# haiciyang/LaDiffCodec

Hardware: AMD Instinct MI355X
Metric: audio-sec decoded / wall-sec, 16kHz 3kbps 50-step DDPM (higher is better)
Workload: dtype bf16; 1 GPU; LaDiffCodec 3 kbps, diff_dims=256, enc_ratios 8 4, 50-step DDPM, batch=32x2.4 s utterances per GPU; global_batch=32, latent_len=1200, denoise_steps=50, rccl_ranks=1, batches_in_flight=1, parallelism=dp1 (utterance-sharded, no data-path collective)

## Files before the change

ladiffcodec_amd/csrc/attention.hip:

```cpp
#include <algorithm>

#include "ldc_kernels.h"
#include "ldc_math.h"

namespace ldc {

__device__ __forceinline__ float abf2f(unsigned short h) { return __uint_as_float(((unsigned)h) << 16); }
__device__ __forceinline__ unsigned short af2bf(float f) { return hw_bf16(f); }
template <typename T>
__device__ __forceinline__ float ld1(const void* p, size_t i);
template <>
__device__ __forceinline__ float ld1<float>(const void* p, size_t i) { return reinterpret_cast<const float*>(p)[i]; }
template <>
__device__ __forceinline__ float ld1<__bf16>(const void* p, size_t i) {
  return abf2f(reinterpret_cast<const unsigned short*>(p)[i]);
}
template <typename T>
__device__ __forceinline__ void st1(void* p, size_t i, float v);
template <>
__device__ __forceinline__ void st1<float>(void* p, size_t i, float v) { reinterpret_cast<float*>(p)[i] = v; }
template <>
__device__ __forceinline__ void st1<__bf16>(void* p, size_t i, float v) {
  reinterpret_cast<unsigned short*>(p)[i] = af2bf(v);
}
// ... 274 lines not shown
    acc = mfma_bf16(af[0], bq[0], acc);
    acc = mfma_bf16(af[1], bq[1], acc);
    if (n < L) {
      unsigned short* orow = out + ((size_t)b * L + n) * HD + h * D;
#pragma unroll
      for (int rr = 0; rr < 4; ++rr) {
        const unsigned lo = (unsigned)af2bf(acc[4 * rr]) | ((unsigned)af2bf(acc[4 * rr + 1]) << 16);
        const unsigned hi = (unsigned)af2bf(acc[4 * rr + 2]) | ((unsigned)af2bf(acc[4 * rr + 3]) << 16);
        *reinterpret_cast<uint2*>(orow + 8 * rr + 4 * g) = n < Lv ? make_uint2(lo, hi) : make_uint2(0u, 0u);
      }
    }
  }
}


__device__ __forceinline__ float reduce16_over32(const float (&v)[16], int lane) {
  float a8[8], a4[4], a2[2];
  const bool b4 = lane & 16, b3 = lane & 8, b2 = lane & 4, b1 = lane & 2;
#pragma unroll
  for (int k = 0; k < 8; ++k) a8[k] = (b4 ? v[8 + k] : v[k]) + __shfl_xor(b4 ? v[k] : v[8 + k], 16);
#pragma unroll
  for (int k = 0; k < 4; ++k) a4[k] = (b3 ? a8[4 + k] : a8[k]) + __shfl_xor(b3 ? a8[k] : a8[4 + k], 8);
#pragma unroll
  for (int k = 0; k < 2; ++k) a2[k] = (b2 ? a4[2 + k] : a4[k]) + __shfl_xor(b2 ? a4[k] : a4[2 + k], 4);
  float a1 = (b1 ? a2[1] : a2[0]) + __shfl_xor(b1 ? a2[0] : a2[1], 2);
  a1 += __shfl_xor(a1, 1);
  return a1;
}

template <int C>
__global__ __launch_bounds__(256) void linattn_tail_mfma_kernel(const unsigned short* qkv, const float* ws, size_t ws_stride, float scale,
                                                                const unsigned short* wo, int n_pad, const float* bias, const float* gain,
                                                                const unsigned short* resid, unsigned short* out, int L, unsigned* fail_flag) {
  constexpr int D = 32, HD = 128, R = 32, CPW = C / 4, NT = CPW / 32;
  constexpr int AP = HD + 8;
  constexpr int TP = CPW * 4 + 16;
  extern __shared__ __attribute__((aligned(16))) char smem[];
  unsigned short* sA = reinterpret_cast<unsigned short*>(smem);
  float* sred = reinterpret_cast<float*>(smem + (size_t)R * AP * 2);
  float* srow = sred + 4 * R;
  char* strans = smem + (size_t)R * AP * 2 + (size_t)5 * R * 4;
  const int b = blockIdx.y, tid = threadIdx.x;
  const int w = tid >> 6, lane = tid & 63, i32 = lane & 31, g = lane >> 5;
  const int r0 = blockIdx.x * R;
  const float* wsb = ws + (size_t)b * ws_stride;
  const int colw = w * CPW + i32;
  uint4 bfr[8][NT];
#pragma unroll
  for (int ks = 0; ks < 8; ++ks)
#pragma unroll
    for (int j = 0; j < NT; ++j)
      bfr[ks][j] = *reinterpret_cast<const uint4*>(wo + ((size_t)(ks >> 1) * n_pad + colw + 32 * j) * 32 + (ks & 1) * 16 + 8 * g);
  float bv[NT], gv[NT];
#pragma unroll
  for (int j = 0; j < NT; ++j) { bv[j] = bias[colw + 32 * j]; gv[j] = gain[colw + 32 * j]; }
  {
    const int h = w;
    const int n = r0 + i32;
    uint4 qq[2];
#pragma unroll
    for (int sx = 0; sx < 2; ++sx) {
      if (n < L) qq[sx] = *reinterpret_cast<const uint4*>(qkv + ((size_t)b * L + n) * (3 * HD) + h * D + 16 * sx + 8 * g);
      else qq[sx] = make_uint4(0, 0, 0, 0);
    }
    uint4 af[2];
    bool ks_bad = false;
#pragma unroll
    for (int sx = 0; sx < 2; ++sx) {
      unsigned wv[4];
#pragma unroll
      for (int m = 0; m < 8; m += 2) {
        const int d0 = 16 * sx + 8 * g + m;
        const float ks0 = wsb[HD + h * D + d0], ks1 = wsb[HD + h * D + d0 + 1];
        ks_bad |= !(ks0 >= kLinattnKsumMin && ks0 < kLinattnKsumMax) | !(ks1 >= kLinattnKsumMin && ks1 < kLinattnKsumMax);
        const float c0 = wsb[2 * HD + (size_t)h * D * D + d0 * D + i32] * (scale / ks0);
        const float c1 = wsb[2 * HD + (size_t)h * D * D + (d0 + 1) * D + i32] * (scale / ks1);
        wv[m >> 1] = (unsigned)af2bf(c0) | ((unsigned)af2bf(c1) << 16);
      }
      af[sx] = make_uint4(wv[0], wv[1], wv[2], wv[3]);
    }
    if (ks_bad && fail_flag) __hip_atomic_store(fail_flag, kDevFailCtxRange, __ATOMIC_RELAXED, __HIP_MEMORY_SCOPE_SYSTEM);
    float x[16];
    float mx = -INFINITY;
#pragma unroll
    for (int sx = 0; sx < 2; ++sx) {
      const unsigned wv[4] = {qq[sx].x, qq[sx].y, qq[sx].z, qq[sx].w};
#pragma unroll
      for (int m = 0; m < 4; ++m) {
        x[8 * sx + 2 * m] = abf2f((unsigned short)(wv[m] & 0xffffu));
        x[8 * sx + 2 * m + 1] = abf2f((unsigned short)(wv[m] >> 16));
      }
    }
#pragma unroll
    for (int m = 0; m < 16; ++m) mx = fmaxf(mx, x[m]);
    mx = fmaxf(mx, __shfl_xor(mx, 32));
    float sum = 0.f;
#pragma unroll
    for (int m = 0; m < 16; ++m) { x[m] = __expf(x[m] - mx); sum += x[m]; }
    sum += __shfl_xor(sum, 32);
    const float inv = 1.0f / sum;
    uint4 bq[2];
#pragma unroll
    for (int sx = 0; sx < 2; ++sx) {
      unsigned wv[4];
#pragma unroll
      for (int m = 0; m < 4; ++m)
        wv[m] = (unsigned)af2bf(x[8 * sx + 2 * m] * inv) | ((unsigned)af2bf(x[8 * sx + 2 * m + 1] * inv) << 16);
      bq[sx] = make_uint4(wv[0], wv[1], wv[2], wv[3]);
    }
    lf32x16 acc1;
#pragma unroll
    for (int r = 0; r < 16; ++r) acc1[r] = 0.f;
    acc1 = mfma_bf16(af[0], bq[0], acc1);
    acc1 = mfma_bf16(af[1], bq[1], acc1);
    unsigned short* arow = sA + (size_t)i32 * AP + h * D;
#pragma unroll
    for (int rr = 0; rr < 4; ++rr) {
      const unsigned lo = (unsigned)af2bf(acc1[4 * rr]) | ((unsigned)af2bf(acc1[4 * rr + 1]) << 16);
      const unsigned hi = (unsigned)af2bf(acc1[4 * rr + 2]) | ((unsigned)af2bf(acc1[4 * rr + 3]) << 16);
      *reinterpret_cast<uint2*>(arow + 8 * rr + 4 * g) = make_uint2(lo, hi);
    }
  }
  __syncthreads();
  lf32x16 acc[NT];
#pragma unroll
  for (int j = 0; j < NT; ++j)
#pragma unroll
    for (int r = 0; r < 16; ++r) acc[j][r] = 0.f;
#pragma unroll
  for (int ks = 0; ks < 8; ++ks) {
    const uint4 afr = *reinterpret_cast<const uint4*>(sA + (size_t)i32 * AP + 16 * ks + 8 * g);
#pragma unroll
    for (int j = 0; j < NT; ++j) acc[j] = mfma_bf16(afr, bfr[ks][j], acc[j]);
  }
  constexpr int LPR = CPW / 4;
  constexpr int RPS = 64 / LPR;
  constexpr int NSW = R / RPS;
  const int rsub = lane / LPR, piece = lane % LPR;
  uint2 rres[NSW];
#pragma unroll
  for (int sw = 0; sw < NSW; ++sw) {
    const int n = r0 + sw * RPS + rsub;
    rres[sw] = n < L ? *reinterpret_cast<const uint2*>(resid + ((size_t)b * L + n) * C + w * CPW + piece * 4) : make_uint2(0, 0);
  }
#pragma unroll
  for (int j = 0; j < NT; ++j)
#pragma unroll
    for (int r = 0; r < 16; ++r) acc[j][r] += bv[j];
  const int rr = i32 >> 1;
  const int my_row = (rr & 3) + 8 * (rr >> 2) + 4 * g;
  {
    float v[16];
#pragma unroll
    for (int r = 0; r < 16; ++r) {
      float sacc = 0.f;
#pragma unroll
      for (int j = 0; j < NT; ++j) sacc += acc[j][r];
      v[r] = sacc;
    }
    const float tot = reduce16_over32(v, lane);
    if ((lane & 1) == 0) sred[w * R + my_row] = tot;
  }
  __syncthreads();
  if (tid < R) srow[tid] = (sred[tid] + sred[R + tid] + sred[2 * R + tid] + sred[3 * R + tid]) * (1.0f / (float)C);
  __syncthreads();
  float mean[16];
#pragma unroll
  for (int r = 0; r < 16; ++r) mean[r] = srow[(r & 3) + 8 * (r >> 2) + 4 * g];
  {
    float v[16];
#pragma unroll
    for (int r = 0; r < 16; ++r) {
      float sacc = 0.f;
#pragma unroll
      for (int j = 0; j < NT; ++j) { const float d = acc[j][r] - mean[r]; sacc = fmaf(d, d, sacc); }
      v[r] = sacc;
    }
    const float tot = reduce16_over32(v, lane);
    if ((lane & 1) == 0) sred[w * R + my_row] = tot;
  }
  __syncthreads();
  if (tid < R) srow[tid] = rsqrtf((sred[tid] + sred[R + tid] + sred[2 * R + tid] + sred[3 * R + tid]) * (1.0f / (float)C) + 1e-5f);
  __syncthreads();
  char* tw = strans + (size_t)w * R * TP;
#pragma unroll
  for (int r = 0; r < 16; ++r) {
    const int row = (r & 3) + 8 * (r >> 2) + 4 * g;
    const float rstd = srow[row];
#pragma unroll
    for (int j = 0; j < NT; ++j)
      reinterpret_cast<float*>(tw + (size_t)row * TP)[32 * j + i32] = (acc[j][r] - mean[r]) * rstd * gv[j];
  }
#pragma unroll
  for (int sw = 0; sw < NSW; ++sw) {
    const int row = sw * RPS + rsub;
    const int n = r0 + row;
    const float4 y = *reinterpret_cast<const float4*>(tw + (size_t)row * TP + piece * 16);
    const float o0 = y.x + abf2f((unsigned short)(rres[sw].x & 0xffffu)), o1 = y.y + abf2f((unsigned short)(rres[sw].x >> 16));
    const float o2 = y.z + abf2f((unsigned short)(rres[sw].y & 0xffffu)), o3 = y.w + abf2f((unsigned short)(rres[sw].y >> 16));
    const uint2 o = make_uint2((unsigned)af2bf(o0) | ((unsigned)af2bf(o1) << 16), (unsigned)af2bf(o2) | ((unsigned)af2bf(o3) << 16));
    if (n < L) *reinterpret_cast<uint2*>(out + ((size_t)b * L + n) * C + w * CPW + piece * 4) = o;
  }
}

template <int C>
static hipError_t launch_tail_cfg(const void* qkv, const float* ws, size_t wss, float scale, const void* wo, int n_pad, const float* bias,
                                  const float* gain, const void* resid, void* out, int B, int L, unsigned* fail_flag, hipStream_t s) {
  constexpr int R = 32, CPW = C / 4;
  const size_t lds = (size_t)R * (128 + 8) * 2 + (size_t)5 * R * 4 + (size_t)4 * R * (CPW * 4 + 16);
  auto kern = linattn_tail_mfma_kernel<C>;
  static bool lds_opt_in = false;
  if (!lds_opt_in) {
    hipError_t e = hipFuncSetAttribute(reinterpret_cast<const void*>(kern), hipFuncAttributeMaxDynamicSharedMemorySize, 160 * 1024);
    if (e != hipSuccess) return e;
    lds_opt_in = true;
  }
  hipLaunchKernelGGL(kern, dim3((L + R - 1) / R, B), dim3(256), lds, s, reinterpret_cast<const unsigned short*>(qkv), ws, wss, scale,
                     reinterpret_cast<const unsigned short*>(wo), n_pad, bias, gain, reinterpret_cast<const unsigned short*>(resid),
                     reinterpret_cast<unsigned short*>(out), L, fail_flag);
  return hipGetLastError();
}

bool linattn_tail_supported(int dt, int heads, int dim_head, int C) {
  return dt == DT_BF16 && heads == 4 && dim_head == 32 && (C == 256 || C == 512 || C == 1024);
}

hipError_t launch_linattn_ctx(int dt, const void* qkv, float* ws, int B, int L, int heads, int dim_head, hipStream_t s) {
  if (dt != DT_BF16 || heads != 4 || dim_head != 32) return hipErrorInvalidValue;
  const size_t wss = linattn_ws_per_item(heads, dim_head);
  hipLaunchKernelGGL(linattn_ctx_mfma_kernel<64>, dim3((L + 63) / 64, B), dim3(256), 0, s, reinterpret_cast<const unsigned short*>(qkv), ws, L, wss,
                     static_cast<const int*>(nullptr), 0);
  return hipGetLastError();
}

hipError_t launch_linattn_tail(int dt, const void* qkv, const float* ws, const void* wo_packed, int n_pad, const float* bias, const float* gain,
                               const void* resid, void* out, int B, int L, int heads, int dim_head, int C, unsigned* fail_flag, hipStream_t s) {
  if (!linattn_tail_supported(dt, heads, dim_head, C) || !bias || !gain || !resid) return hipErrorInvalidValue;
  const size_t wss = linattn_ws_per_item(heads, dim_head);
  const float scale = 1.0f / sqrtf((float)dim_head);
  if (C == 256) return launch_tail_cfg<256>(qkv, ws, wss, scale, wo_packed, n_pad, bias, gain, resid, out, B, L, fail_flag, s);
  if (C == 512) return launch_tail_cfg<512>(qkv, ws, wss, scale, wo_packed, n_pad, bias, gain, resid, out, B, L, fail_flag, s);
  return launch_tail_cfg<1024>(qkv, ws, wss, scale, wo_packed, n_pad, bias, gain, resid, out, B, L, fail_flag, s);
}

size_t linattn_ws_floats_per_item(int heads, int dim_head) { return linattn_ws_per_item(heads, dim_head); }

hipError_t launch_linattn_kmax(int dt, const void* qkv, float* ws, int B, int L, int heads, int dim_head, hipStream_t s, const int* lens, int shift) {
  const int HD = heads * dim_head;
  if (dim_head != 32 || HD > 256 || 256 % HD) return hipErrorInvalidValue;
  const size_t wss = linattn_ws_per_item(heads, dim_head);
  hipError_t e = hipMemsetAsync(ws, 0, (size_t)B * wss * sizeof(float), s);
  if (e != hipSuccess) return e;
  const int rpb = 128;
  if (dt == DT_F32) hipLaunchKernelGGL(linattn_kmax_kernel<float>, dim3((L + rpb - 1) / rpb, B), dim3(256), 0, s, qkv, ws, L, HD, rpb, wss, lens, shift);
  else hipLaunchKernelGGL(linattn_kmax_kernel<__bf16>, dim3((L + rpb - 1) / rpb, B), dim3(256), 0, s, qkv, ws, L, HD, rpb, wss, lens, shift);
  return hipGetLastError();
}
// ... 130 lines not shown
```

ladiffcodec_amd/csrc/ldc_api.cpp:

```cpp
#include "ldc_internal.h"

long long g_device_syncs = 0;

static thread_local char g_err[1024] = "";
int fail(int code, const char* fmt, ...) {
  va_list ap;
  va_start(ap, fmt);
  vsnprintf(g_err, sizeof(g_err), fmt, ap);
  va_end(ap);
  return code;
}

extern "C" const char* ldc_last_error(void) { return g_err; }
extern "C" const char* ldc_version(void) { return "ladiffcodec-amd 0.1 (gfx950)"; }



static std::vector<float> fold_weight_norm(const HostTensor& g, const HostTensor& v) {
  const size_t n0 = (size_t)v.shape[0], inner = v.numel() / n0;
  std::vector<float> w(v.numel());
  for (size_t i = 0; i < n0; ++i) {
    double s = 0;
    for (size_t j = 0; j < inner; ++j) s += (double)v.data[i * inner + j] * v.data[i * inner + j];
    const float nrm = (float)sqrt(s);
// ... 780 lines not shown
  LDC_OPT("ends_join", c->ends_join, false, 0, 1)
  LDC_OPT("split_init", c->split_init, true, 0, 1)
  LDC_OPT("side_streams", c->side_streams, true, 0, 1)
  LDC_OPT("serial_parts", c->serial_parts, false, 0, 1)
  LDC_OPT("stream_calib", c->calib, false, 0, 1)
  LDC_OPT("merge_advance", c->merge_advance, true, 0, 1)
  LDC_OPT("fuse_gn_stats", c->fuse_gn_stats, true, 0, 1)
  LDC_OPT("fuse_gn_epi", c->fuse_gn_epi, true, 0, 1)
  LDC_OPT("gn_epi_min_l", c->gn_epi_min_l, true, 0, 1 << 30)
  LDC_OPT("gn_epi_max_tiles", c->gn_epi_max_tiles, true, 0, 1 << 30)
  LDC_OPT("fold_res", c->fold_res, true, 0, 1)
  LDC_OPT("fold_ln", c->fold_ln, true, 0, 1)
  LDC_OPT("fuse_kmax", c->fuse_kmax, true, 0, 1)
  LDC_OPT("fuse_ln", c->fuse_ln, true, 0, 1)
  LDC_OPT("fuse_attn_tail", c->fuse_attn_tail, true, 0, 1)
  LDC_OPT("fold_ctx", c->fold_ctx, true, 0, 1)
  LDC_OPT("conv_lean", c->tune.lean, true, 0, 1)
  LDC_OPT("lean_all", c->tune.lean_all, true, 0, 1)
  LDC_OPT("ring3_tiles", c->tune.ring3_tiles, true, 0, 1 << 30)
  LDC_OPT("ring3_wgs", c->tune.ring3_wgs, true, 1, 3)
  LDC_OPT("ring3_window", c->tune.ring3_window, true, 0, 1)
  LDC_OPT("ring3_window_tiles", c->tune.ring3_window_tiles, true, 0, 1 << 30)
  LDC_OPT("conv_generic", c->tune.force_generic, true, 0, 1)
  LDC_OPT("conv_small_tiles", c->tune.small_max, true, 0, 1 << 30)
  LDC_OPT("conv_splitk", c->tune.splitk, true, 0, 4)
  LDC_OPT("sk_tiles", c->tune.sk_tiles, true, 0, 1 << 30)
  LDC_OPT("sk_u2", c->tune.sk_u2, true, 0, 1 << 30)
  LDC_OPT("sk_u3", c->tune.sk_u3, true, 0, 1 << 30)
  LDC_OPT("conv_mfast", c->tune.m_fastest, true, 0, 2)
  LDC_OPT("conv_debug", c->tune.debug, true, 0, 255)
// ... 1543 lines not shown
```

ladiffcodec_amd/csrc/ldc_api_tuning.cpp:

```cpp
#include "ldc_internal.h"

static int round_up(int v, int m) { return (v + m - 1) / m * m; }

extern "C" int ldc_sconv1d(ldc_ctx* c, const float* x, int B, int Cin, int L, const float* w_host, const float* b_host,
                           int Cout, int k, int stride, int dilation, int causal, int pre_elu, float* y, void* stream) {
  if (!c || !x || !w_host || !y) return fail(LDC_E_INVALID, "null argument");
  if (B <= 0 || Cin <= 0 || L <= 0 || Cout <= 0 || k <= 0 || stride <= 0 || dilation <= 0) return fail(LDC_E_INVALID, "bad sizes");
  HIPCHK(hipSetDevice(c->device));
  hipStream_t s = pick_stream(c, stream);
  const int cp = round_up(Cin, 16);
  std::vector<float> wp((size_t)Cout * cp * k, 0.f);
  for (int o = 0; o < Cout; ++o)
    for (int i = 0; i < Cin; ++i)
      for (int t = 0; t < k; ++t) wp[((size_t)o * cp + i) * k + t] = w_host[((size_t)o * Cin + i) * k + t];
  DevMem keep;
  std::swap(keep.ptrs, c->wmem.ptrs);
  ConvLayer ly;
  ConvSpec sp;
  sp.dt = DT_F32; sp.cin1 = cp; sp.cout = Cout; sp.k = k; sp.stride = stride; sp.dil = dilation;
  const int padding_total = (k - 1) * dilation - (stride - 1);
  sp.pad_left = causal ? padding_total : padding_total - padding_total / 2;
  sp.pad_mode = PAD_REFLECT; sp.pre_act = pre_elu ? ACT_ELU : ACT_NONE;
  int rc = make_conv(c, sp, wp.data(), b_host, &ly);
  std::swap(keep.ptrs, c->wmem.ptrs);
// ... 698 lines not shown
    std::swap(keep.ptrs, c->wmem.ptrs);
    c->w8 = saved_w8;
    LDCCHK(rc);
    LDCCHK(keep.alloc(&r_cl, (size_t)B * L * C * es));
    HIPCHK(launch_to_cl(dt, resid, r_cl, B, C, L, nullptr, 0, 0.f, s));
  }
  HIPCHK(launch_to_cl(dt, qkv, q_cl, B, 3 * HD, L, nullptr, 0, 0.f, s));
  if (kind == 0) {
    HIPCHK(launch_linattn(dt, q_cl, o_cl, (float*)ws, B, L, H, D, false, s));
  } else if (kind == 1) {
    HIPCHK(launch_linattn_kmax(dt, q_cl, (float*)ws, B, L, H, D, s));
    HIPCHK(launch_linattn(dt, q_cl, o_cl, (float*)ws, B, L, H, D, true, s));
  } else if (kind == 2) {
    HIPCHK(launch_linattn_kmax(dt, q_cl, (float*)ws, B, L, H, D, s));
    HIPCHK(launch_linattn_ctx(dt, q_cl, (float*)ws, B, L, H, D, s));
    HIPCHK(launch_linattn_tail(dt, q_cl, (const float*)ws, to_out.w, to_out.n_pad, to_out.bias, d_gain, r_cl, o_cl, B, L, H, D, C, c->dev_flag_dev, s));
  } else {
    HIPCHK(launch_attn_full(dt, q_cl, o_cl, B, L, H, D, s));
  }
  HIPCHK(launch_from_cl(dt, o_cl, out, B, Co, L, nullptr, 0, 0.f, s));
  HIPCHK(hipStreamSynchronize(s));
  return check_dev_flag(c);
}

extern "C" int ldc_conv_compare_fp8(ldc_ctx* c, int B, int L, int cin1, int cin2, int cout, int k, int stride, int ups, int with_gn,
                                    int with_colmax, double* max_abs_diff, double* max_abs_ref, double* max_rel_stat) {
  if (!c || !max_abs_diff || !max_abs_ref || !max_rel_stat) return fail(LDC_E_INVALID, "bad arguments");
  if ((cin1 % 64) || (cin2 % 64)) return fail(LDC_E_INVALID, "fp8 inputs need channel counts that are multiples of 64");
  HIPCHK(hipSetDevice(c->device));
  const int cin = cin1 + cin2;
  std::vector<float> w((size_t)cout * cin * k), bias(cout);
// ... 242 lines not shown
```

ladiffcodec_amd/csrc/ldc_internal.h:

```cpp
#pragma once
#include "../../include/ladiffcodec.h"

#include <hip/hip_runtime.h>
#include <math.h>
#include <stdarg.h>
#include <stdio.h>
#include <string.h>

#include <algorithm>
#include <chrono>
#include <functional>
#include <map>
#include <memory>
#include <set>
#include <string>
#include <vector>

#include "ldc_kernels.h"
#include "ldc_windows.h"
#include "plan_passes.h"
static_assert(kGnSumFloats == ldc::kGnPad, "plan_passes.h sizes the GroupNorm sums by the kernels' padding");

extern long long g_device_syncs;
inline hipError_t counted_device_sync() {
// ... 240 lines not shown
  int fp8_act = 1;
  int part_graphs = 1;
  double host_graph_ms = 0, host_wait_ms = 0;
  long long host_graph_launches = 0;
  hipStream_t side_stream[kMaxParts] = {nullptr, nullptr, nullptr, nullptr};
  hipEvent_t ev_side_fork[kMaxParts] = {nullptr, nullptr, nullptr, nullptr}, ev_side_join[kMaxParts] = {nullptr, nullptr, nullptr, nullptr};
  int side_streams = 0;
  int fuse_kmax = 1;
  int fuse_ln = 1;
  int coop_launch = 0;
  int lstm_xcd = 1;
  int num_cus = 256;
  int xcd_resident[2] = {0, 0};
  int coop_resident[2] = {0, 0};
  int fuse_attn_tail = 1;
  int fold_ctx = 1;
  static constexpr int kFlowRing = 32;
  hipEvent_t flow_ev[kFlowRing] = {};
  unsigned long long flow_n = 0;
  int flow_depth = 8;
  int fuse_gn_stats = 1;
  int gn_epi_max_tiles = 1300;
  int gn_epi_min_l = 0;
  int fold_ln = 1;
  int fold_res = 1;
  int fuse_gn_epi = 1;
  ConvTune tune;
  int lstm_stream_only = 0;
  int serial_parts = 0;
  int graph_steps = 0;
// ... 191 lines not shown
```

ladiffcodec_amd/csrc/ldc_kernels.h:

```cpp
#pragma once
#include <hip/hip_runtime.h>
#include <stdint.h>

#include "ldc_windows.h"

namespace ldc {

enum { DT_F32 = 0, DT_BF16 = 1, DT_FP8 = 2 };
enum { ACT_NONE = 0, ACT_SILU = 1, ACT_ELU = 2, ACT_TANH = 3, ACT_GELU = 4, ACT_SIGMOID = 5, ACT_RELU = 6 };
enum { PAD_ZERO = 0, PAD_REFLECT = 1 };
static constexpr int kGnPad = 16;

inline size_t dt_size(int dt) { return dt == DT_F32 ? 4 : (dt == DT_FP8 ? 1 : 2); }

struct ConvLayer {
  int dt = DT_F32;
  int cin1 = 0, cin2 = 0;
  int n = 0;
  int n_pad = 0;
  int bn = 128;
  int taps = 1, stride = 1, dil = 1, pad_left = 0, ups = 0, pad_mode = PAD_ZERO;
  int pre_act = ACT_NONE, post_act = ACT_NONE;
  int tr_stride = 0, tr_cout = 0, tr_trim_left = 0;
  void* w = nullptr;
// ... 88 lines not shown
                           int ss_stride, const int* t_ptr, int act, hipStream_t s, void* y_ln = nullptr, const float* ln_g = nullptr, int out8 = 0,
                           const int* lens = nullptr, int shift = 0,
                           int t_stride = 0, int t_rows = 0);
bool gn_apply_ln_fusable(int C);
hipError_t launch_ln_rows(int dt, const void* x, void* y, const void* residual, const float* g, int rows, int C,
                          hipStream_t s, int out8 = 0, const int* lens = nullptr, int shift = 0, int L = 0);
hipError_t launch_mask_rows(int dt, void* x, int B, int L, int C, const int* lens, int shift, hipStream_t s);
hipError_t launch_act(int dt, const void* x, void* y, int64_t n, int act, hipStream_t s, int out8 = 0);

hipError_t launch_linattn(int dt, const void* qkv, void* out, float* ctx_ws, int B, int L, int heads, int dim_head,
                          bool kmax_fused, hipStream_t s, const int* lens = nullptr, int shift = 0, bool ws_zeroed = false);
size_t linattn_ws_floats_per_item(int heads, int dim_head);
bool linattn_tail_supported(int dt, int heads, int dim_head, int C);
hipError_t launch_linattn_ctx(int dt, const void* qkv, float* ctx_ws, int B, int L, int heads, int dim_head, hipStream_t s);
hipError_t launch_linattn_tail(int dt, const void* qkv, const float* ctx_ws, const void* wo_packed, int n_pad, const float* bias, const float* gain,
                               const void* resid, void* out, int B, int L, int heads, int dim_head, int C, unsigned* fail_flag, hipStream_t s);
hipError_t launch_linattn_kmax(int dt, const void* qkv, float* ctx_ws, int B, int L, int heads, int dim_head, hipStream_t s,
                               const int* lens = nullptr, int shift = 0);
constexpr float kLinattnKClamp = 60.0f;
constexpr float kLinattnKsumMin = 7.888609052210118e-31f;
constexpr float kLinattnKsumMax = 1.0e26f;
constexpr unsigned kDevFailCtxRange = 4u;
hipError_t launch_attn_full(int dt, const void* qkv, void* out, int B, int L, int heads, int dim_head, hipStream_t s, const int* lens = nullptr,
                            int shift = 0);

hipError_t launch_to_cl(int dt, const float* x_bcl, void* y_blc, int B, int C, int L, const float* maxabs,
                        int maxabs_per_item, float eps, hipStream_t s);
hipError_t launch_from_cl(int dt, const void* x_blc, float* y_bcl, int B, int C, int L, const float* maxabs,
                          int maxabs_per_item, float eps, hipStream_t s);
hipError_t launch_maxabs(int dt, const void* x, int B, int64_t n_per_item, int per_item, float* maxabs,
                         hipStream_t s);
// ... 192 lines not shown
```

ladiffcodec_amd/csrc/unet_plan.cpp:

```cpp
#include "ldc_internal.h"

bool gn_apply_fp8_ok(int C) { return C % 8 == 0 && C / 8 <= 256 && 256 % (C / 8) == 0 && C <= 2048; }

void* PlanBuilder::act(int rows, int C) {
  pl->act_bytes += (double)rows * C * es;
  return ar->alloc((size_t)rows * C * es);
}
const int* PlanBuilder::lens() const { return pl->ragged ? (pl->lens ? pl->lens : reinterpret_cast<const int*>(16)) : nullptr; }
int PlanBuilder::level(int L) const {
  int sh = 0;
  while ((L << sh) < pl->L) ++sh;
  return sh;
}
void PlanBuilder::mask(void* y, int L, int C) {
  if (!pl->ragged) return;
  const int dt = c->dt, Bn = B, sh = level(L);
  const int* ln = pl->lens;
  info = "mask_rows_c" + std::to_string(C) + "_L" + std::to_string(L);
  add([=](hipStream_t s) { return launch_mask_rows(dt, y, Bn, L, C, ln, sh, s); }, false, 0, LDC_CLASS_ELEMENTWISE, 0);
}
void PlanBuilder::mark(int kind) {
  pl->step.push_back({[](hipStream_t) { return hipSuccess; }, kind, LDC_CLASS_OTHER, 0, 0, "-"});
}
void PlanBuilder::add(std::function<hipError_t(hipStream_t)> f, bool is_conv, double flops, int cls, double bytes) {
// ... 212 lines not shown
        2.0 * rows * a.dim * es);
  if (linear) {
    const size_t wss = linattn_ws_floats_per_item(H, Dh);
    if (!ln && c->fuse_kmax && c->fuse_attn_tail && !a.out.w8 && linattn_tail_supported(dt, H, Dh, a.dim)) {
      ln_rowstat_next = rowstat;
      if (lnf && c->fold_ctx && c->tune.lean && !c->tune.force_generic && dt == DT_BF16 && a.qkv_ctx.w && hid == 128 && a.dim % 64 == 0) {
        qkv_ctx_next = ws; qkv_ctx_stride_next = (int)wss;
        conv(a.qkv_ctx, xn, nullptr, qkv, nullptr, L, L);
      } else {
        conv(qkv_ly, xn, nullptr, qkv, nullptr, L, L, nullptr, reinterpret_cast<unsigned*>(ws), hid, 2 * hid, (int)wss);
        add([=](hipStream_t s) { return launch_linattn_ctx(dt, qkv, ws, Bn, L, H, Dh, s); }, false, 0, LDC_CLASS_LINATTN, 2.0 * rows * hid * es);
      }
      const int dim = a.dim;
      info = "tail_c" + std::to_string(dim) + "_L" + std::to_string(L) + "_B" + std::to_string(B);
      unsigned* flag = c->dev_flag_dev;
      add([=](hipStream_t s) {
        return launch_linattn_tail(dt, qkv, ws, ap->out.w, ap->out.n_pad, ap->out.bias, ap->out_g, x, out, Bn, L, H, Dh, dim, flag, s);
      }, false, 2.0 * rows * hid * dim, LDC_CLASS_LINATTN, (1.0 * hid + 2.0 * dim) * rows * es);
      return out;
    }
    if (c->fuse_kmax && !ln) {
      ln_rowstat_next = rowstat;
      conv(qkv_ly, xn, nullptr, qkv, nullptr, L, L, nullptr, reinterpret_cast<unsigned*>(ws), hid, 2 * hid, (int)wss);
      add([=](hipStream_t s) { return launch_linattn(dt, qkv, o, ws, Bn, L, H, Dh, true, s); }, false, 0, LDC_CLASS_LINATTN,
          4.0 * rows * hid * es);
    } else {
      ln_rowstat_next = rowstat;
      conv(qkv_ly, xn, nullptr, qkv, nullptr, L, L);
      add([=](hipStream_t s) { return launch_linattn(dt, qkv, o, ws, Bn, L, H, Dh, false, s, ln, sh, ln != nullptr); }, false, 0, LDC_CLASS_LINATTN,
          5.0 * rows * hid * es);
    }
    void* t = act(rows, a.dim);
// ... 302 lines not shown
```

Before: 654.7 audio-s/wall-s.

## Make linear-attention tail kernel persistent with 8 waves and reused weight registers

The fused linear-attention output tail kernel now uses 512-thread workgroups (8 waves splitting the output channels) and a persistent grid. Each workgroup walks a run of (batch, row-block) pairs, so the to_out weight fragments, bias and gain stay in registers across rows instead of being reloaded per 32-row block. The next block's Q is prefetched and residual loads are issued early. Context normalisation also now loads one ksum per lane and broadcasts it by shuffle. The run length comes from occupancy queries, with an optional override knob and compile-time timestamp instrumentation, at the cost of more register pressure and a grid sized to residency.

```diff
diff --git a/ladiffcodec_amd/csrc/attention.hip b/ladiffcodec_amd/csrc/attention.hip
--- a/ladiffcodec_amd/csrc/attention.hip
+++ b/ladiffcodec_amd/csrc/attention.hip
@@ -1,4 +1,7 @@
 #include <algorithm>
+#include <climits>
+#include <cstdio>
+#include <vector>
 
 #include "ldc_kernels.h"
 #include "ldc_math.h"
@@ -312,6 +315,27 @@
 }
 
 
+#ifndef LDC_TAIL_STAMPS
+#define LDC_TAIL_STAMPS 0
+#endif
+
+constexpr int kTailWaves = 8, kTailRows = 32;
+template <int C>
+struct TailLds {
+  static constexpr int AP = 128 + 8;
+  static constexpr int TP = (C / kTailWaves) * 4 + 16;
+  static constexpr size_t red = (size_t)kTailRows * AP * 2;
+  static constexpr size_t mean = red + (size_t)kTailWaves * kTailRows * 4;
+  static constexpr size_t rstd = mean + (size_t)kTailRows * 4;
+  static constexpr size_t trans = rstd + (size_t)kTailRows * 4;
+  static constexpr size_t bytes = trans + (size_t)kTailWaves * kTailRows * TP;
+  static_assert(trans % 16 == 0 && TP % 16 == 0, "16-byte pieces of the transpose region");
+  static_assert(bytes <= (size_t)160 * 1024, "one workgroup must fit a CU's LDS");
+};
+template <int C>
+constexpr size_t tail_lds_bytes() { return TailLds<C>::bytes; }
+static_assert(tail_lds_bytes<256>() == 46848 && tail_lds_bytes<512>() == 79616 && tail_lds_bytes<1024>() == 145152, "tail LDS layout");
+
 __device__ __forceinline__ float reduce16_over32(const float (&v)[16], int lane) {
   float a8[8], a4[4], a2[2];
   const bool b4 = lane & 16, b3 = lane & 8, b2 = lane & 4, b1 = lane & 2;
@@ -326,197 +350,307 @@
   return a1;
 }
 
+__device__ __forceinline__ void tail_load_q(const unsigned short* qkv, int b, int r0, int L, int h, int lane, uint4 (&qq)[2]) {
+  const int n = r0 + (lane & 31), g = lane >> 5;
+#pragma unroll
+  for (int sx = 0; sx < 2; ++sx) {
+    if (n < L) qq[sx] = *reinterpret_cast<const uint4*>(qkv + ((size_t)b * L + n) * (3 * 128) + h * 32 + 16 * sx + 8 * g);
+    else qq[sx] = make_uint4(0, 0, 0, 0);
+  }
+}
+__device__ __forceinline__ void tail_context_operand(const float* wsb, int h, int lane, float scale, unsigned* fail_flag, uint4 (&af)[2]) {
+  const int i32 = lane & 31, g = lane >> 5;
+  const float ksv = wsb[128 + h * 32 + i32];
+  float craw[16];
+#pragma unroll
+  for (int sx = 0; sx < 2; ++sx)
+#pragma unroll
+    for (int m = 0; m < 8; ++m) craw[8 * sx + m] = wsb[2 * 128 + (size_t)h * 32 * 32 + (16 * sx + 8 * g + m) * 32 + i32];
+  const bool ks_bad = !(ksv >= kLinattnKsumMin && ksv < kLinattnKsumMax);
+  if (ks_bad && fail_flag) __hip_atomic_store(fail_flag, kDevFailCtxRange, __ATOMIC_RELAXED, __HIP_MEMORY_SCOPE_SYSTEM);
+  const float sk = scale / ksv;
+#pragma unroll
+  for (int sx = 0; sx < 2; ++sx) {
+    unsigned wv[4];
+#pragma unroll
+    for (int m = 0; m < 8; m += 2) {
+      const int d0 = 16 * sx + 8 * g + m;
+      const float c0 = craw[8 * sx + m] * __shfl(sk, d0);
+      const float c1 = craw[8 * sx + m + 1] * __shfl(sk, d0 + 1);
+      wv[m >> 1] = (unsigned)af2bf(c0) | ((unsigned)af2bf(c1) << 16);
+    }
+    af[sx] = make_uint4(wv[0], wv[1], wv[2], wv[3]);
+  }
+}
+
 template <int C>
-__global__ __launch_bounds__(256) void linattn_tail_mfma_kernel(const unsigned short* qkv, const float* ws, size_t ws_stride, float scale,
+__global__ __launch_bounds__(512, C == 256 ? 4 : 2) void linattn_tail_mfma_kernel(const unsigned short* qkv, const float* ws, size_t ws_stride, float scale,
                                                                 const unsigned short* wo, int n_pad, const float* bias, const float* gain,
-                                                                const unsigned short* resid, unsigned short* out, int L, unsigned* fail_flag) {
-  constexpr int D = 32, HD = 128, R = 32, CPW = C / 4, NT = CPW / 32;
-  constexpr int AP = HD + 8;
-  constexpr int TP = CPW * 4 + 16;
+                                                                const unsigned short* resid, unsigned short* out, int L, int nblk, int npairs,
+                                                                int nb, unsigned* fail_flag, unsigned long long* stamps) {
+  constexpr int D = 32, HD = 128, R = kTailRows, CPW = C / kTailWaves, NT = CPW / 32;
+  using Lds = TailLds<C>;
+  constexpr int AP = Lds::AP, TP = Lds::TP;
+  constexpr bool kResidAhead = C <= 512;
   extern __shared__ __attribute__((aligned(16))) char smem[];
   unsigned short* sA = reinterpret_cast<unsigned short*>(smem);
-  float* sred = reinterpret_cast<float*>(smem + (size_t)R * AP * 2);
-  float* srow = sred + 4 * R;
-  char* strans = smem + (size_t)R * AP * 2 + (size_t)5 * R * 4;
-  const int b = blockIdx.y, tid = threadIdx.x;
-  const int w = tid >> 6, lane = tid & 63, i32 = lane & 31, g = lane >> 5;
-  const int r0 = blockIdx.x * R;
-  const float* wsb = ws + (size_t)b * ws_stride;
-  const int colw = w * CPW + i32;
+  float* sred = reinterpret_cast<float*>(smem + Lds::red);
+  float* smean = reinterpret_cast<float*>(smem + Lds::mean);
+  float* srstd = reinterpret_cast<float*>(smem + Lds::rstd);
+  char* strans = smem + Lds::trans;
+  const int tid = threadIdx.x;
+  const int w = __builtin_amdgcn_readfirstlane(tid >> 6), lane0 = tid & 63;
+  const int colw = w * CPW + (lane0 & 31);
+  unsigned long long tst[6] = {0, 0, 0, 0, 0, 0};
+  if (LDC_TAIL_STAMPS) tst[0] = __builtin_amdgcn_s_memtime();
   uint4 bfr[8][NT];
 #pragma unroll
   for (int ks = 0; ks < 8; ++ks)
 #pragma unroll
     for (int j = 0; j < NT; ++j)
-      bfr[ks][j] = *reinterpret_cast<const uint4*>(wo + ((size_t)(ks >> 1) * n_pad + colw + 32 * j) * 32 + (ks & 1) * 16 + 8 * g);
+      bfr[ks][j] = *reinterpret_cast<const uint4*>(wo + ((size_t)(ks >> 1) * n_pad + colw + 32 * j) * 32 + (ks & 1) * 16 + 8 * (lane0 >> 5));
   float bv[NT], gv[NT];
 #pragma unroll
   for (int j = 0; j < NT; ++j) { bv[j] = bias[colw + 32 * j]; gv[j] = gain[colw + 32 * j]; }
-  {
-    const int h = w;
-    const int n = r0 + i32;
-    uint4 qq[2];
-#pragma unroll
-    for (int sx = 0; sx < 2; ++sx) {
-      if (n < L) qq[sx] = *reinterpret_cast<const uint4*>(qkv + ((size_t)b * L + n) * (3 * HD) + h * D + 16 * sx + 8 * g);
-      else qq[sx] = make_uint4(0, 0, 0, 0);
-    }
-    uint4 af[2];
-    bool ks_bad = false;
-#pragma unroll
-    for (int sx = 0; sx < 2; ++sx) {
-      unsigned wv[4];
-#pragma unroll
-      for (int m = 0; m < 8; m += 2) {
-        const int d0 = 16 * sx + 8 * g + m;
-        const float ks0 = wsb[HD + h * D + d0], ks1 = wsb[HD + h * D + d0 + 1];
-        ks_bad |= !(ks0 >= kLinattnKsumMin && ks0 < kLinattnKsumMax) | !(ks1 >= kLinattnKsumMin && ks1 < kLinattnKsumMax);
-        const float c0 = wsb[2 * HD + (size_t)h * D * D + d0 * D + i32] * (scale / ks0);
-        const float c1 = wsb[2 * HD + (size_t)h * D * D + (d0 + 1) * D + i32] * (scale / ks1);
-        wv[m >> 1] = (unsigned)af2bf(c0) | ((unsigned)af2bf(c1) << 16);
-      }
-      af[sx] = make_uint4(wv[0], wv[1], wv[2], wv[3]);
-    }
-    if (ks_bad && fail_flag) __hip_atomic_store(fail_flag, kDevFailCtxRange, __ATOMIC_RELAXED, __HIP_MEMORY_SCOPE_SYSTEM);
-    float x[16];
-    float mx = -INFINITY;
-#pragma unroll
-    for (int sx = 0; sx < 2; ++sx) {
-      const unsigned wv[4] = {qq[sx].x, qq[sx].y, qq[sx].z, qq[sx].w};
-#pragma unroll
-      for (int m = 0; m < 4; ++m) {
-        x[8 * sx + 2 * m] = abf2f((unsigned short)(wv[m] & 0xffffu));
-        x[8 * sx + 2 * m + 1] = abf2f((unsigned short)(wv[m] >> 16));
-      }
-    }
-#pragma unroll
-    for (int m = 0; m < 16; ++m) mx = fmaxf(mx, x[m]);
-    mx = fmaxf(mx, __shfl_xor(mx, 32));
-    float sum = 0.f;
-#pragma unroll
-    for (int m = 0; m < 16; ++m) { x[m] = __expf(x[m] - mx); sum += x[m]; }
-    sum += __shfl_xor(sum, 32);
-    const float inv = 1.0f / sum;
-    uint4 bq[2];
-#pragma unroll
-    for (int sx = 0; sx < 2; ++sx) {
-      unsigned wv[4];
-#pragma unroll
-      for (int m = 0; m < 4; ++m)
-        wv[m] = (unsigned)af2bf(x[8 * sx + 2 * m] * inv) | ((unsigned)af2bf(x[8 * sx + 2 * m + 1] * inv) << 16);
-      bq[sx] = make_uint4(wv[0], wv[1], wv[2], wv[3]);
-    }
-    lf32x16 acc1;
-#pragma unroll
-    for (int r = 0; r < 16; ++r) acc1[r] = 0.f;
-    acc1 = mfma_bf16(af[0], bq[0], acc1);
-    acc1 = mfma_bf16(af[1], bq[1], acc1);
-    unsigned short* arow = sA + (size_t)i32 * AP + h * D;
-#pragma unroll
-    for (int rr = 0; rr < 4; ++rr) {
-      const unsigned lo = (unsigned)af2bf(acc1[4 * rr]) | ((unsigned)af2bf(acc1[4 * rr + 1]) << 16);
-      const unsigned hi = (unsigned)af2bf(acc1[4 * rr + 2]) | ((unsigned)af2bf(acc1[4 * rr + 3]) << 16);
-      *reinterpret_cast<uint2*>(arow + 8 * rr + 4 * g) = make_uint2(lo, hi);
-    }
-  }
-  __syncthreads();
-  lf32x16 acc[NT];
-#pragma unroll
-  for (int j = 0; j < NT; ++j)
-#pragma unroll
-    for (int r = 0; r < 16; ++r) acc[j][r] = 0.f;
-#pragma unroll
-  for (int ks = 0; ks < 8; ++ks) {
-    const uint4 afr = *reinterpret_cast<const uint4*>(sA + (size_t)i32 * AP + 16 * ks + 8 * g);
-#pragma unroll
-    for (int j = 0; j < NT; ++j) acc[j] = mfma_bf16(afr, bfr[ks][j], acc[j]);
-  }
-  constexpr int LPR = CPW / 4;
-  constexpr int RPS = 64 / LPR;
-  constexpr int NSW = R / RPS;
-  const int rsub = lane / LPR, piece = lane % LPR;
-  uint2 rres[NSW];
-#pragma unroll
-  for (int sw = 0; sw < NSW; ++sw) {
-    const int n = r0 + sw * RPS + rsub;
-    rres[sw] = n < L ? *reinterpret_cast<const uint2*>(resid + ((size_t)b * L + n) * C + w * CPW + piece * 4) : make_uint2(0, 0);
-  }
-#pragma unroll
-  for (int j = 0; j < NT; ++j)
-#pragma unroll
-    for (int r = 0; r < 16; ++r) acc[j][r] += bv[j];
-  const int rr = i32 >> 1;
-  const int my_row = (rr & 3) + 8 * (rr >> 2) + 4 * g;
-  {
-    float v[16];
+  if (LDC_TAIL_STAMPS) { asm volatile("s_waitcnt vmcnt(0)" ::: "memory"); tst[1] = __builtin_amdgcn_s_memtime(); }
+  const int p0 = blockIdx.x * nb, p1 = min(p0 + nb, npairs);
+  int b = p0 / nblk, r0 = (p0 - b * nblk) * R;
+  uint4 qq[2], af[2];
+  if (w < 4) {
+    tail_load_q(qkv, b, r0, L, w, lane0, qq);
+    tail_context_operand(ws + (size_t)b * ws_stride, w, lane0, scale, fail_flag, af);
+  }
+#pragma unroll 1
+  for (int p = p0; p < p1; ++p) {
+    int lane = lane0;
+    asm volatile("" : "+v"(lane));
+    const int i32 = lane & 31, g = lane >> 5;
+    if (w < 4) {
+      const int h = w;
+      float x[16];
+      float mx = -INFINITY;
+#pragma unroll
+      for (int sx = 0; sx < 2; ++sx) {
+        const unsigned wv[4] = {qq[sx].x, qq[sx].y, qq[sx].z, qq[sx].w};
+#pragma unroll
+        for (int m = 0; m < 4; ++m) {
+          x[8 * sx + 2 * m] = abf2f((unsigned short)(wv[m] & 0xffffu));
+          x[8 * sx + 2 * m + 1] = abf2f((unsigned short)(wv[m] >> 16));
+        }
+      }
+#pragma unroll
+      for (int m = 0; m < 16; ++m) mx = fmaxf(mx, x[m]);
+      mx = fmaxf(mx, __shfl_xor(mx, 32));
+      float sum = 0.f;
+#pragma unroll
+      for (int m = 0; m < 16; ++m) { x[m] = __expf(x[m] - mx); sum += x[m]; }
+      sum += __shfl_xor(sum, 32);
+      const float inv = 1.0f / sum;
+      uint4 bq[2];
+#pragma unroll
+      for (int sx = 0; sx < 2; ++sx) {
+        unsigned wv[4];
+#pragma unroll
+        for (int m = 0; m < 4; ++m)
+          wv[m] = (unsigned)af2bf(x[8 * sx + 2 * m] * inv) | ((unsigned)af2bf(x[8 * sx + 2 * m + 1] * inv) << 16);
+        bq[sx] = make_uint4(wv[0], wv[1], wv[2], wv[3]);
+      }
+      lf32x16 acc1;
+#pragma unroll
+      for (int r = 0; r < 16; ++r) acc1[r] = 0.f;
+      acc1 = mfma_bf16(af[0], bq[0], acc1);
+      acc1 = mfma_bf16(af[1], bq[1], acc1);
+      unsigned short* arow = sA + (size_t)i32 * AP + h * D;
+#pragma unroll
+      for (int rr = 0; rr < 4; ++rr) {
+        const unsigned lo = (unsigned)af2bf(acc1[4 * rr]) | ((unsigned)af2bf(acc1[4 * rr + 1]) << 16);
+        const unsigned hi = (unsigned)af2bf(acc1[4 * rr + 2]) | ((unsigned)af2bf(acc1[4 * rr + 3]) << 16);
+        *reinterpret_cast<uint2*>(arow + 8 * rr + 4 * g) = make_uint2(lo, hi);
+      }
+    }
+    __syncthreads();
+    if (LDC_TAIL_STAMPS) tst[2] = __builtin_amdgcn_s_memtime();
+    lf32x16 acc[NT];
+#pragma unroll
+    for (int j = 0; j < NT; ++j)
+#pragma unroll
+      for (int r = 0; r < 16; ++r) acc[j][r] = 0.f;
+#pragma unroll
+    for (int ks = 0; ks < 8; ++ks) {
+      const uint4 afr = *reinterpret_cast<const uint4*>(sA + (size_t)i32 * AP + 16 * ks + 8 * g);
+#pragma unroll
+      for (int j = 0; j < NT; ++j) acc[j] = mfma_bf16(afr, bfr[ks][j], acc[j]);
+    }
+    constexpr int LPR = CPW / 4;
+    constexpr int RPS = 64 / LPR;
+    constexpr int NSW = R / RPS;
+    const int rsub = lane / LPR, piece = lane % LPR;
+    constexpr int NSA = kResidAhead ? NSW : 0;
+    uint2 rres[NSW];
+    auto load_resid = [&](int sw) {
+      const int n = r0 + sw * RPS + rsub;
+      rres[sw] = n < L ? *reinterpret_cast<const uint2*>(resid + ((size_t)b * L + n) * C + w * CPW + piece * 4) : make_uint2(0, 0);
+    };
+#pragma unroll
+    for (int sw = 0; sw < NSA; ++sw) load_resid(sw);
+    int bn = b, rn = r0 + R;
+    if (rn >= L) { bn = b + 1; rn = 0; }
+    const bool more = p + 1 < p1;
+    if (more && w < 4) tail_load_q(qkv, bn, rn, L, w, lane, qq);
+    if (LDC_TAIL_STAMPS) tst[3] = __builtin_amdgcn_s_memtime();
+#pragma unroll
+    for (int j = 0; j < NT; ++j)
+#pragma unroll
+      for (int r = 0; r < 16; ++r) acc[j][r] += bv[j];
+    const int rr = i32 >> 1;
+    const int my_row = (rr & 3) + 8 * (rr >> 2) + 4 * g;
+    {
+      float v[16];
+#pragma unroll
+      for (int r = 0; r < 16; ++r) {
+        float sacc = 0.f;
+#pragma unroll
+        for (int j = 0; j < NT; ++j) sacc += acc[j][r];
+        v[r] = sacc;
+      }
+      const float tot = reduce16_over32(v, lane);
+      if ((lane & 1) == 0) sred[w * R + my_row] = tot;
+    }
+    __syncthreads();
+    if (tid < R) {
+      float t = sred[tid];
+#pragma unroll
+      for (int k = 1; k < kTailWaves; ++k) t += sred[k * R + tid];
+      smean[tid] = t * (1.0f / (float)C);
+    }
+    __syncthreads();
+    {
+      float v[16];
+#pragma unroll
+      for (int r = 0; r < 16; ++r) {
+        const float mean = smean[(r & 3) + 8 * (r >> 2) + 4 * g];
+        float sacc = 0.f;
+#pragma unroll
+        for (int j = 0; j < NT; ++j) { const float d = acc[j][r] - mean; sacc = fmaf(d, d, sacc); }
+        v[r] = sacc;
+      }
+      const float tot = reduce16_over32(v, lane);
+      if ((lane & 1) == 0) sred[w * R + my_row] = tot;
+    }
+    __syncthreads();
+    if (tid < R) {
+      float t = sred[tid];
+#pragma unroll
+      for (int k = 1; k < kTailWaves; ++k) t += sred[k * R + tid];
+      srstd[tid] = rsqrtf(t * (1.0f / (float)C) + 1e-5f);
+    }
+    __syncthreads();
+    if (LDC_TAIL_STAMPS) tst[4] = __builtin_amdgcn_s_memtime();
+    char* tw = strans + (size_t)w * R * TP;
 #pragma unroll
     for (int r = 0; r < 16; ++r) {
-      float sacc = 0.f;
-#pragma unroll
-      for (int j = 0; j < NT; ++j) sacc += acc[j][r];
-      v[r] = sacc;
-    }
-    const float tot = reduce16_over32(v, lane);
-    if ((lane & 1) == 0) sred[w * R + my_row] = tot;
-  }
-  __syncthreads();
-  if (tid < R) srow[tid] = (sred[tid] + sred[R + tid] + sred[2 * R + tid] + sred[3 * R + tid]) * (1.0f / (float)C);
-  __syncthreads();
-  float mean[16];
-#pragma unroll
-  for (int r = 0; r < 16; ++r) mean[r] = srow[(r & 3) + 8 * (r >> 2) + 4 * g];
-  {
-    float v[16];
-#pragma unroll
-    for (int r = 0; r < 16; ++r) {
-      float sacc = 0.f;
-#pragma unroll
-      for (int j = 0; j < NT; ++j) { const float d = acc[j][r] - mean[r]; sacc = fmaf(d, d, sacc); }
-      v[r] = sacc;
-    }
-    const float tot = reduce16_over32(v, lane);
-    if ((lane & 1) == 0) sred[w * R + my_row] = tot;
-  }
-  __syncthreads();
-  if (tid < R) srow[tid] = rsqrtf((sred[tid] + sred[R + tid] + sred[2 * R + tid] + sred[3 * R + tid]) * (1.0f / (float)C) + 1e-5f);
-  __syncthreads();
-  char* tw = strans + (size_t)w * R * TP;
-#pragma unroll
-  for (int r = 0; r < 16; ++r) {
-    const int row = (r & 3) + 8 * (r >> 2) + 4 * g;
-    const float rstd = srow[row];
-#pragma unroll
-    for (int j = 0; j < NT; ++j)
-      reinterpret_cast<float*>(tw + (size_t)row * TP)[32 * j + i32] = (acc[j][r] - mean[r]) * rstd * gv[j];
-  }
-#pragma unroll
-  for (int sw = 0; sw < NSW; ++sw) {
-    const int row = sw * RPS + rsub;
-    const int n = r0 + row;
-    const float4 y = *reinterpret_cast<const float4*>(tw + (size_t)row * TP + piece * 16);
-    const float o0 = y.x + abf2f((unsigned short)(rres[sw].x & 0xffffu)), o1 = y.y + abf2f((unsigned short)(rres[sw].x >> 16));
-    const float o2 = y.z + abf2f((unsigned short)(rres[sw].y & 0xffffu)), o3 = y.w + abf2f((unsigned short)(rres[sw].y >> 16));
-    const uint2 o = make_uint2((unsigned)af2bf(o0) | ((unsigned)af2bf(o1) << 16), (unsigned)af2bf(o2) | ((unsigned)af2bf(o3) << 16));
-    if (n < L) *reinterpret_cast<uint2*>(out + ((size_t)b * L + n) * C + w * CPW + piece * 4) = o;
-  }
+      const int row = (r & 3) + 8 * (r >> 2) + 4 * g;
+      const float mean = smean[row], rstd = srstd[row];
+#pragma unroll
+      for (int j = 0; j < NT; ++j)
+        reinterpret_cast<float*>(tw + (size_t)row * TP)[32 * j + i32] = (acc[j][r] - mean) * rstd * gv[j];
+    }
+#pragma unroll
+    for (int sw = NSA; sw < NSW; ++sw) load_resid(sw);
+#pragma unroll
+    for (int sw = 0; sw < NSW; ++sw) {
+      const int row = sw * RPS + rsub;
+      const int n = r0 + row;
+      const float4 y = *reinterpret_cast<const float4*>(tw + (size_t)row * TP + piece * 16);
+      const float o0 = y.x + abf2f((unsigned short)(rres[sw].x & 0xffffu)), o1 = y.y + abf2f((unsigned short)(rres[sw].x >> 16));
+      const float o2 = y.z + abf2f((unsigned short)(rres[sw].y & 0xffffu)), o3 = y.w + abf2f((unsigned short)(rres[sw].y >> 16));
+      const uint2 o = make_uint2((unsigned)af2bf(o0) | ((unsigned)af2bf(o1) << 16), (unsigned)af2bf(o2) | ((unsigned)af2bf(o3) << 16));
+      if (n < L) *reinterpret_cast<uint2*>(out + ((size_t)b * L + n) * C + w * CPW + piece * 4) = o;
+    }
+    if (more && bn != b && w < 4) tail_context_operand(ws + (size_t)bn * ws_stride, w, lane, scale, fail_flag, af);
+    b = bn; r0 = rn;
+  }
+  if (LDC_TAIL_STAMPS && stamps) {
+    asm volatile("s_waitcnt vmcnt(0)" ::: "memory");
+    tst[5] = __builtin_amdgcn_s_memtime();
+    if (tid == 0)
+      for (int k = 0; k < 6; ++k) stamps[(size_t)blockIdx.x * 6 + k] = tst[k];
+  }
+}
+
+#if LDC_TAIL_STAMPS
+static void tail_stamps_report(const unsigned long long* dev, int grid, int C, int B, int L, int nb) {
+  std::vector<unsigned long long> h((size_t)grid * 6);
+  if (hipMemcpy(h.data(), dev, h.size() * 8, hipMemcpyDeviceToHost) != hipSuccess) return;
+  unsigned long long lo = ~0ull, hi = 0;
+  std::vector<unsigned long long> d[6];
+  for (int i = 0; i < grid; ++i) {
+    const unsigned long long* t = &h[(size_t)i * 6];
+    lo = std::min(lo, t[0]); hi = std::max(hi, t[5]);
+    for (int k = 0; k < 5; ++k) d[k].push_back(t[k + 1] - t[k]);
+    d[5].push_back(t[5] - t[0]);
+  }
+  fprintf(stderr, "TAIL_STAMPS C=%d B=%d L=%d nb=%d grid=%d span=%llu |", C, B, L, nb, grid, hi - lo);
+  const char* nm[6] = {"weights", "phase1", "phase2", "layernorm", "store", "total"};
+  for (int k = 0; k < 6; ++k) {
+    std::sort(d[k].begin(), d[k].end());
+    fprintf(stderr, " %s med %llu max %llu |", nm[k], d[k][d[k].size() / 2], d[k].back());
+  }
+  fprintf(stderr, "\n");
+}
+#endif
+
+struct TailResidency { int wgs = 0, cus = 0; };
+
+static int tail_run_length(int npairs, int run, int C, const TailResidency& res) {
+  if (run >= 1) return run;
+  const int one_round = (npairs + res.wgs - 1) / res.wgs;
+  const int fill = std::max(1, std::min(one_round, npairs / res.cus));
+  const int amortise = std::max(1, (2 * 128 * C) / (128 << 10));
+  return std::max(fill, amortise);
 }
 
 template <int C>
 static hipError_t launch_tail_cfg(const void* qkv, const float* ws, size_t wss, float scale, const void* wo, int n_pad, const float* bias,
-                                  const float* gain, const void* resid, void* out, int B, int L, unsigned* fail_flag, hipStream_t s) {
-  constexpr int R = 32, CPW = C / 4;
-  const size_t lds = (size_t)R * (128 + 8) * 2 + (size_t)5 * R * 4 + (size_t)4 * R * (CPW * 4 + 16);
+                                  const float* gain, const void* resid, void* out, int B, int L, int run, unsigned* fail_flag, hipStream_t s) {
+  constexpr int R = kTailRows, NTHR = 64 * kTailWaves;
+  constexpr size_t lds = tail_lds_bytes<C>();
   auto kern = linattn_tail_mfma_kernel<C>;
-  static bool lds_opt_in = false;
-  if (!lds_opt_in) {
-    hipError_t e = hipFuncSetAttribute(reinterpret_cast<const void*>(kern), hipFuncAttributeMaxDynamicSharedMemorySize, 160 * 1024);
+  static TailResidency res;
+  if (!res.wgs) {
+    hipError_t e = hipFuncSetAttribute(reinterpret_cast<const void*>(kern), hipFuncAttributeMaxDynamicSharedMemorySize, (int)lds);
     if (e != hipSuccess) return e;
-    lds_opt_in = true;
-  }
-  hipLaunchKernelGGL(kern, dim3((L + R - 1) / R, B), dim3(256), lds, s, reinterpret_cast<const unsigned short*>(qkv), ws, wss, scale,
+    int dev = 0, cus = 0, occ = 0;
+    if ((e = hipGetDevice(&dev)) != hipSuccess) return e;
+    if ((e = hipDeviceGetAttribute(&cus, hipDeviceAttributeMultiprocessorCount, dev)) != hipSuccess) return e;
+    if ((e = hipOccupancyMaxActiveBlocksPerMultiprocessor(&occ, kern, NTHR, lds)) != hipSuccess) return e;
+    if (occ < 1 || cus < 1) return hipErrorLaunchOutOfResources;
+    res.cus = cus;
+    res.wgs = occ * cus;
+  }
+  const int nblk = (L + R - 1) / R;
+  const long long np = (long long)B * nblk;
+  if (np > INT_MAX) return hipErrorInvalidValue;
+  const int npairs = (int)np, nb = std::min(npairs, tail_run_length(npairs, run, C, res)), grid = (npairs + nb - 1) / nb;
+  unsigned long long* stamps = nullptr;
+#if LDC_TAIL_STAMPS
+  static unsigned long long* stamp_buf = nullptr;
+  static int stamp_cap = 0;
+  if (grid > stamp_cap) {
+    if (stamp_buf) (void)hipFree(stamp_buf);
+    if (hipMalloc((void**)&stamp_buf, (size_t)grid * 6 * 8) != hipSuccess) return hipErrorOutOfMemory;
+    stamp_cap = grid;
+  }
+  stamps = stamp_buf;
+#endif
+  hipLaunchKernelGGL(kern, dim3(grid), dim3(NTHR), lds, s, reinterpret_cast<const unsigned short*>(qkv), ws, wss, scale,
                      reinterpret_cast<const unsigned short*>(wo), n_pad, bias, gain, reinterpret_cast<const unsigned short*>(resid),
-                     reinterpret_cast<unsigned short*>(out), L, fail_flag);
-  return hipGetLastError();
+                     reinterpret_cast<unsigned short*>(out), L, nblk, npairs, nb, fail_flag, stamps);
+  hipError_t e = hipGetLastError();
+#if LDC_TAIL_STAMPS
+  if (e == hipSuccess && (e = hipStreamSynchronize(s)) == hipSuccess) tail_stamps_report(stamps, grid, C, B, L, nb);
+#endif
+  return e;
 }
 
 bool linattn_tail_supported(int dt, int heads, int dim_head, int C) {
@@ -532,13 +666,13 @@
 }
 
 hipError_t launch_linattn_tail(int dt, const void* qkv, const float* ws, const void* wo_packed, int n_pad, const float* bias, const float* gain,
-                               const void* resid, void* out, int B, int L, int heads, int dim_head, int C, unsigned* fail_flag, hipStream_t s) {
-  if (!linattn_tail_supported(dt, heads, dim_head, C) || !bias || !gain || !resid) return hipErrorInvalidValue;
+                               const void* resid, void* out, int B, int L, int heads, int dim_head, int C, unsigned* fail_flag, hipStream_t s, int run) {
+  if (!linattn_tail_supported(dt, heads, dim_head, C) || !bias || !gain || !resid || run < 0) return hipErrorInvalidValue;
   const size_t wss = linattn_ws_per_item(heads, dim_head);
   const float scale = 1.0f / sqrtf((float)dim_head);
-  if (C == 256) return launch_tail_cfg<256>(qkv, ws, wss, scale, wo_packed, n_pad, bias, gain, resid, out, B, L, fail_flag, s);
-  if (C == 512) return launch_tail_cfg<512>(qkv, ws, wss, scale, wo_packed, n_pad, bias, gain, resid, out, B, L, fail_flag, s);
-  return launch_tail_cfg<1024>(qkv, ws, wss, scale, wo_packed, n_pad, bias, gain, resid, out, B, L, fail_flag, s);
+  if (C == 256) return launch_tail_cfg<256>(qkv, ws, wss, scale, wo_packed, n_pad, bias, gain, resid, out, B, L, run, fail_flag, s);
+  if (C == 512) return launch_tail_cfg<512>(qkv, ws, wss, scale, wo_packed, n_pad, bias, gain, resid, out, B, L, run, fail_flag, s);
+  return launch_tail_cfg<1024>(qkv, ws, wss, scale, wo_packed, n_pad, bias, gain, resid, out, B, L, run, fail_flag, s);
 }
 
 size_t linattn_ws_floats_per_item(int heads, int dim_head) { return linattn_ws_per_item(heads, dim_head); }
diff --git a/ladiffcodec_amd/csrc/ldc_api.cpp b/ladiffcodec_amd/csrc/ldc_api.cpp
--- a/ladiffcodec_amd/csrc/ldc_api.cpp
+++ b/ladiffcodec_amd/csrc/ldc_api.cpp
@@ -818,6 +818,7 @@
   LDC_OPT("fuse_kmax", c->fuse_kmax, true, 0, 1)
   LDC_OPT("fuse_ln", c->fuse_ln, true, 0, 1)
   LDC_OPT("fuse_attn_tail", c->fuse_attn_tail, true, 0, 1)
+  LDC_OPT("attn_tail_run", c->attn_tail_run, true, 0, 1 << 20)
   LDC_OPT("fold_ctx", c->fold_ctx, true, 0, 1)
   LDC_OPT("conv_lean", c->tune.lean, true, 0, 1)
   LDC_OPT("lean_all", c->tune.lean_all, true, 0, 1)
diff --git a/ladiffcodec_amd/csrc/ldc_api_tuning.cpp b/ladiffcodec_amd/csrc/ldc_api_tuning.cpp
--- a/ladiffcodec_amd/csrc/ldc_api_tuning.cpp
+++ b/ladiffcodec_amd/csrc/ldc_api_tuning.cpp
@@ -736,7 +736,8 @@
   } else if (kind == 2) {
     HIPCHK(launch_linattn_kmax(dt, q_cl, (float*)ws, B, L, H, D, s));
     HIPCHK(launch_linattn_ctx(dt, q_cl, (float*)ws, B, L, H, D, s));
-    HIPCHK(launch_linattn_tail(dt, q_cl, (const float*)ws, to_out.w, to_out.n_pad, to_out.bias, d_gain, r_cl, o_cl, B, L, H, D, C, c->dev_flag_dev, s));
+    HIPCHK(launch_linattn_tail(dt, q_cl, (const float*)ws, to_out.w, to_out.n_pad, to_out.bias, d_gain, r_cl, o_cl, B, L, H, D, C, c->dev_flag_dev, s,
+                               c->attn_tail_run));
   } else {
     HIPCHK(launch_attn_full(dt, q_cl, o_cl, B, L, H, D, s));
   }
diff --git a/ladiffcodec_amd/csrc/ldc_internal.h b/ladiffcodec_amd/csrc/ldc_internal.h
--- a/ladiffcodec_amd/csrc/ldc_internal.h
+++ b/ladiffcodec_amd/csrc/ldc_internal.h
@@ -278,6 +278,7 @@
   int xcd_resident[2] = {0, 0};
   int coop_resident[2] = {0, 0};
   int fuse_attn_tail = 1;
+  int attn_tail_run = 0;
   int fold_ctx = 1;
   static constexpr int kFlowRing = 32;
   hipEvent_t flow_ev[kFlowRing] = {};
diff --git a/ladiffcodec_amd/csrc/ldc_kernels.h b/ladiffcodec_amd/csrc/ldc_kernels.h
--- a/ladiffcodec_amd/csrc/ldc_kernels.h
+++ b/ladiffcodec_amd/csrc/ldc_kernels.h
@@ -126,7 +126,8 @@
 bool linattn_tail_supported(int dt, int heads, int dim_head, int C);
 hipError_t launch_linattn_ctx(int dt, const void* qkv, float* ctx_ws, int B, int L, int heads, int dim_head, hipStream_t s);
 hipError_t launch_linattn_tail(int dt, const void* qkv, const float* ctx_ws, const void* wo_packed, int n_pad, const float* bias, const float* gain,
-                               const void* resid, void* out, int B, int L, int heads, int dim_head, int C, unsigned* fail_flag, hipStream_t s);
+                               const void* resid, void* out, int B, int L, int heads, int dim_head, int C, unsigned* fail_flag, hipStream_t s,
+                               int run = 0);
 hipError_t launch_linattn_kmax(int dt, const void* qkv, float* ctx_ws, int B, int L, int heads, int dim_head, hipStream_t s,
                                const int* lens = nullptr, int shift = 0);
 constexpr float kLinattnKClamp = 60.0f;
diff --git a/ladiffcodec_amd/csrc/unet_plan.cpp b/ladiffcodec_amd/csrc/unet_plan.cpp
--- a/ladiffcodec_amd/csrc/unet_plan.cpp
+++ b/ladiffcodec_amd/csrc/unet_plan.cpp
@@ -250,8 +250,9 @@
       const int dim = a.dim;
       info = "tail_c" + std::to_string(dim) + "_L" + std::to_string(L) + "_B" + std::to_string(B);
       unsigned* flag = c->dev_flag_dev;
+      const int run = c->attn_tail_run;
       add([=](hipStream_t s) {
-        return launch_linattn_tail(dt, qkv, ws, ap->out.w, ap->out.n_pad, ap->out.bias, ap->out_g, x, out, Bn, L, H, Dh, dim, flag, s);
+        return launch_linattn_tail(dt, qkv, ws, ap->out.w, ap->out.n_pad, ap->out.bias, ap->out_g, x, out, Bn, L, H, Dh, dim, flag, s, run);
       }, false, 2.0 * rows * hid * dim, LDC_CLASS_LINATTN, (1.0 * hid + 2.0 * dim) * rows * es);
       return out;
     }
```

Measured after the change: 659.8 audio-s/wall-s (median of 6 runs). About the same (+0.8%).
